# NVlabs/VILA

Measured on NVIDIA H100. Metric: NVILA-8B decode tokens/sec (1 img 448^2, bs=1, 128 new tokens); TTFT reported as ttft_ms, higher is better.
Workload: dtype bf16

## Files before the change

### vila_b200/csrc/gemm_wgmma.cu

```cuda
#include "common.cuh"
#include "kernels.h"
#include "wgmma.cuh"

namespace vb {

namespace {

constexpr int BLOCK_M = 128;
constexpr int BLOCK_K = 64;
constexpr int kConsumerThreads = 256;
constexpr int kNumThreads = kConsumerThreads + 32;

enum { kModeSingle = 0, kModePair = 1, kModeSplitK2 = 2 };

template <int BLOCK_N, int kStages, int kMode = kModeSingle>
struct GemmSmem {
  static constexpr int kABytes = BLOCK_M * BLOCK_K * 2;
  static constexpr int kBBytes = BLOCK_N * BLOCK_K * 2;
  static constexpr int kStageBytes = kABytes + kBBytes;
  static constexpr int kBarrierBytes = 2 * kStages * 8 + 16;
  static constexpr int kTotal = kStages * kStageBytes + kBarrierBytes + 1024;
  static_assert(kMode != kModeSplitK2 || BLOCK_M * BLOCK_N * 2 <= kStages * kStageBytes, "");
};

__device__ __forceinline__ float2 ld_cg_v2(const float* p) {
  float2 r;
  asm volatile("ld.global.cg.v2.f32 {%0,%1}, [%2];" : "=f"(r.x), "=f"(r.y) : "l"(p));
  return r;
}

constexpr int kBandM = 8;
__device__ __forceinline__ void tile_coords(int t, int num_m_blocks, int num_n_blocks, int& m_blk, int& n_blk) {
  const int per_band = kBandM * num_n_blocks;
  const int band = t / per_band;
  const int r = t - band * per_band;
  const int m0 = band * kBandM;
  const int bm = min(kBandM, num_m_blocks - m0);
  n_blk = r / bm;
  m_blk = m0 + (r - n_blk * bm);
}

struct Sched {
  int nkb, num_m_blocks, num_tiles;
  int stream_k;
  long it, it_end;
  int tile;
  int stride;
  __device__ __forceinline__ Sched(int M, int N, int K, int block_n, int stream_k_, int tile_m,
                                   int worker, int n_workers) {
    nkb = (K + BLOCK_K - 1) / BLOCK_K;
    num_m_blocks = (M + tile_m - 1) / tile_m;
    num_tiles = num_m_blocks * ((N + block_n - 1) / block_n);
    stream_k = stream_k_;
    const long total = static_cast<long>(num_tiles) * nkb;
    it = total * worker / n_workers;
    it_end = total * (worker + 1) / n_workers;
    tile = worker;
    stride = n_workers;
  }
  __device__ __forceinline__ bool next(int& t, int& kb0, int& kb1) {
    if (stream_k) {
      if (it >= it_end) return false;
      t = static_cast<int>(it / nkb);
      kb0 = static_cast<int>(it - static_cast<long>(t) * nkb);
      const long rem = it_end - it;
      kb1 = (nkb - kb0) < rem ? nkb : kb0 + static_cast<int>(rem);
      it += kb1 - kb0;
      return true;
    }
    if (tile >= num_tiles) return false;
    t = tile;
    kb0 = 0;
    kb1 = nkb;
    tile += stride;
    return true;
  }
};

template <int BLOCK_N>
__device__ __forceinline__ void epilogue_store(const float* acc, const GemmEpilogue& epi, __nv_bfloat16* C,
                                               int ldc, int M, int N, int row0, int n_base, int col0,
                                               int j_lo, int j_hi) {
#pragma unroll
  for (int h = 0; h < 2; ++h) {
    const int row = row0 + 8 * h;
    if (row >= M) continue;
    const __nv_bfloat16* res_row = nullptr;
    if (epi.residual != nullptr) {
      const int rr = epi.res_row_mod > 0 ? (row % epi.res_row_mod) : row;
      res_row = epi.residual + static_cast<size_t>(rr) * epi.ld_res;
    }
#pragma unroll
    for (int j = 0; j < BLOCK_N / 8; ++j) {
      if (j < j_lo || j >= j_hi) continue;
      const int n = n_base + 8 * j + col0;
      if (n >= N) continue;
      float v0 = acc[4 * j + 2 * h], v1 = acc[4 * j + 2 * h + 1];
      if (epi.bias != nullptr) {
        const uint32_t b = *reinterpret_cast<const uint32_t*>(epi.bias + n);
        v0 += bf_lo(b);
        v1 += bf_hi(b);
      }
      if (epi.swiglu) {
        const float g = bf16_round(v0), u = bf16_round(v1);
        C[static_cast<size_t>(row) * ldc + (n >> 1)] = __float2bfloat16_rn(bf16_round(silu_f(g)) * u);
        continue;
      }
      if (epi.act != ACT_NONE) {
        const float x0 = bf16_round(v0), x1 = bf16_round(v1);
        if (epi.act == ACT_GELU_TANH) {
          v0 = gelu_tanh_f(x0);
          v1 = gelu_tanh_f(x1);
        } else if (epi.act == ACT_GELU_ERF) {
          v0 = gelu_erf_f(x0);
          v1 = gelu_erf_f(x1);
        } else {
          v0 = silu_f(x0);
          v1 = silu_f(x1);
        }
      }
      if (res_row != nullptr) {
        const uint32_t r = *reinterpret_cast<const uint32_t*>(res_row + n);
        v0 = bf16_round(v0) + bf_lo(r);
        v1 = bf16_round(v1) + bf_hi(r);
      }
      *reinterpret_cast<uint32_t*>(C + static_cast<size_t>(row) * ldc + n) = pack_bf16(v0, v1);
    }
  }
}

template <int BLOCK_N, int kStages, int kMode>
__global__ void __launch_bounds__(kNumThreads, 1)
gemm_bf16_wgmma_kernel(const __grid_constant__ CUtensorMap tmap_a,
                       const __grid_constant__ CUtensorMap tmap_w, __nv_bfloat16* __restrict__ C,
                       int ldc, int M, int N, int K, GemmEpilogue epi) {
  using S = GemmSmem<BLOCK_N, kStages, kMode>;
  constexpr bool kPair = kMode == kModePair;
  constexpr bool kSplit2 = kMode == kModeSplitK2;
  constexpr bool kCluster = kPair || kSplit2;
  constexpr int TILE_M = kPair ? 2 * BLOCK_M : BLOCK_M;
  constexpr int kAcc = BLOCK_N / 2;
  extern __shared__ uint8_t smem_raw[];
  uint8_t* smem = reinterpret_cast<uint8_t*>((reinterpret_cast<uintptr_t>(smem_raw) + 1023) &
                                             ~static_cast<uintptr_t>(1023));
  uint8_t* smem_a = smem;
  uint8_t* smem_b = smem + kStages * S::kABytes;
  uint64_t* full_bar = reinterpret_cast<uint64_t*>(smem + kStages * S::kStageBytes);
  uint64_t* empty_bar = full_bar + kStages;
  uint32_t* last_flag = reinterpret_cast<uint32_t*>(empty_bar + kStages);

  const int warp = threadIdx.x >> 5;
  const int lane = threadIdx.x & 31;
  const int num_m_blocks = (M + TILE_M - 1) / TILE_M;
  const int num_n_blocks = (N + BLOCK_N - 1) / BLOCK_N;
  const int stream_k = (!kCluster && epi.split_k > 1) ? 1 : 0;
  const uint32_t rank = kCluster ? cluster_ctarank() : 0u;
  const uint32_t mrank = kPair ? rank : 0u;
  const int worker = kCluster ? static_cast<int>(blockIdx.x >> 1) : static_cast<int>(blockIdx.x);
  const int n_workers = kCluster ? static_cast<int>(gridDim.x >> 1) : static_cast<int>(gridDim.x);
  const int nkb_all = (K + BLOCK_K - 1) / BLOCK_K;
  const int sk_lo = (kSplit2 && rank == 1) ? (nkb_all + 1) / 2 : 0;
  const int sk_hi = (kSplit2 && rank == 0) ? (nkb_all + 1) / 2 : nkb_all;

  if (threadIdx.x == kConsumerThreads) {
    tma_prefetch_desc(&tmap_a);
    tma_prefetch_desc(&tmap_w);
#pragma unroll
    for (int i = 0; i < kStages; ++i) {
      mbar_init(&full_bar[i], 1);
      mbar_init(&empty_bar[i], kPair ? 4 : 2);
    }
    fence_barrier_init();
  }
  if (kCluster) cluster_sync_all();
  else __syncthreads();
  griddep_launch_dependents();

  if (warp == kConsumerThreads / 32) {
    if (lane == 0) {
      Sched sch(M, N, K, BLOCK_N, stream_k, TILE_M, worker, n_workers);
      constexpr int kWRows = kPair ? BLOCK_N / 2 : BLOCK_N;
      const int a_row_off = static_cast<int>(mrank) * BLOCK_M;
      const int w_row_off = static_cast<int>(mrank) * kWRows;
      auto load_w = [&](int stage, int kb, int n_blk) {
        uint8_t* dst = smem_b + stage * S::kBBytes + w_row_off * (BLOCK_K * 2);
        if (kPair) tma_load_2d_multicast(dst, &tmap_w, &full_bar[stage], kb * BLOCK_K, n_blk * BLOCK_N + w_row_off, 3);
        else tma_load_2d(dst, &tmap_w, &full_bar[stage], kb * BLOCK_K, n_blk * BLOCK_N);
      };
      int stage = 0;
      uint32_t phase = 0;
      int t, kb0, kb1;
      int pre = 0;
      int pt = 0, pkb0 = 0, pkb1 = 0;
      Sched peek = sch;
      const bool have_first = peek.next(pt, pkb0, pkb1);
      if (kSplit2) {
        pkb0 = sk_lo;
        pkb1 = sk_hi;
      }
      if (!kPair && epi.static_w && have_first) {
        pre = min(kStages, pkb1 - pkb0);
        int m_blk_unused, n_blk;
        tile_coords(pt, num_m_blocks, num_n_blocks, m_blk_unused, n_blk);
        for (int i = 0; i < pre; ++i) {
          mbar_arrive_expect_tx(&full_bar[i], S::kStageBytes);
          load_w(i, pkb0 + i, n_blk);
        }
      }
      griddep_wait();
      bool first = true;
      while (sch.next(t, kb0, kb1)) {
        int m_blk, n_blk;
        tile_coords(t, num_m_blocks, num_n_blocks, m_blk, n_blk);
        if (kSplit2) {
          kb0 = sk_lo;
          kb1 = sk_hi;
        }
        for (int kb = kb0; kb < kb1; ++kb) {
          if (first && (kb - kb0) < pre) {
            tma_load_2d(smem_a + stage * S::kABytes, &tmap_a, &full_bar[stage], kb * BLOCK_K,
                        m_blk * TILE_M + a_row_off);
          } else {
            mbar_wait(&empty_bar[stage], phase ^ 1);
            mbar_arrive_expect_tx(&full_bar[stage], S::kStageBytes);
            tma_load_2d(smem_a + stage * S::kABytes, &tmap_a, &full_bar[stage], kb * BLOCK_K,
                        m_blk * TILE_M + a_row_off);
            load_w(stage, kb, n_blk);
          }
          if (++stage == kStages) {
            stage = 0;
            phase ^= 1;
          }
        }
        first = false;
      }
    }
  } else {
    const int wg = warp >> 2;
    const int ctid = threadIdx.x;
    const int frag_row = wg * 64 + (warp & 3) * 16 + (lane >> 2);
    const int col0 = (lane & 3) * 2;
    Sched sch(M, N, K, BLOCK_N, stream_k, TILE_M, worker, n_workers);
    int stage = 0;
    uint32_t phase = 0;
    int t, kb0, kb1;
    float acc[kAcc];
    griddep_wait();
    while (sch.next(t, kb0, kb1)) {
      int m_blk, n_blk;
      tile_coords(t, num_m_blocks, num_n_blocks, m_blk, n_blk);
      if (kSplit2) {
        kb0 = sk_lo;
        kb1 = sk_hi;
      }
      auto release = [&](int s) {
        __syncwarp();
        if ((warp & 3) == 0 && lane == 0) {
          if (kPair) {
            mbar_arrive_cluster(mapa_u32(smem_u32(&empty_bar[s]), 0));
            mbar_arrive_cluster(mapa_u32(smem_u32(&empty_bar[s]), 1));
          } else {
            mbar_arrive(&empty_bar[s]);
          }
        }
      };
      int prev_stage = -1;
      for (int kb = kb0; kb < kb1; ++kb) {
        mbar_wait(&full_bar[stage], phase);
        wgmma_fence_operand<kAcc>(acc);
        wgmma_fence();
        const uint32_t a_base = smem_u32(smem_a + stage * S::kABytes) + wg * (64 * BLOCK_K * 2);
        const uint32_t b_base = smem_u32(smem_b + stage * S::kBBytes);
#pragma unroll
        for (int k = 0; k < BLOCK_K / 16; ++k) {
          const uint64_t ad = make_wgmma_desc(a_base + k * 32, 16, 1024, kWgmmaSW128);
          const uint64_t bd = make_wgmma_desc(b_base + k * 32, 16, 1024, kWgmmaSW128);
          Wgmma<BLOCK_N>::ss(acc, ad, bd, (kb != kb0 || k != 0) ? 1u : 0u);
        }
        wgmma_commit();
        wgmma_wait<1>();
        wgmma_fence_operand<kAcc>(acc);
        if (prev_stage >= 0) release(prev_stage);
        prev_stage = stage;
        if (++stage == kStages) {
          stage = 0;
          phase ^= 1;
        }
      }
      wgmma_wait<0>();
      wgmma_fence_operand<kAcc>(acc);
      if (prev_stage >= 0) release(prev_stage);

      const int row0 = m_blk * TILE_M + static_cast<int>(mrank) * BLOCK_M + frag_row;
      const int n_base = n_blk * BLOCK_N;
      int j_lo = 0, j_hi = BLOCK_N / 8;
      if (kSplit2) {
        named_bar_sync(1, kConsumerThreads);
        float2* xchg = reinterpret_cast<float2*>(smem_a);
        constexpr int kHalfJ = BLOCK_N / 16;
        const bool mine_low = rank == 0;
#pragma unroll
        for (int j = 0; j < BLOCK_N / 8; ++j) {
          if ((j < kHalfJ) == mine_low) continue;
#pragma unroll
          for (int h = 0; h < 2; ++h)
            xchg[((j % kHalfJ) * 2 + h) * kConsumerThreads + ctid] =
                make_float2(acc[4 * j + 2 * h], acc[4 * j + 2 * h + 1]);
        }
        cluster_sync_all();
        const uint32_t xchg_peer = mapa_u32(smem_u32(xchg), 1u - rank);
        j_lo = static_cast<int>(rank) * kHalfJ;
        j_hi = j_lo + kHalfJ;
#pragma unroll
        for (int j = 0; j < BLOCK_N / 8; ++j) {
          if ((j < kHalfJ) != mine_low) continue;
#pragma unroll
          for (int h = 0; h < 2; ++h) {
            const float2 q =
                ld_dsmem_v2f(xchg_peer + static_cast<uint32_t>(((j % kHalfJ) * 2 + h) * kConsumerThreads + ctid) * 8u);
            acc[4 * j + 2 * h] += q.x;
            acc[4 * j + 2 * h + 1] += q.y;
          }
        }
      }
      const bool partial = stream_k && ((kb0 != 0) || (kb1 != sch.nkb));
      bool finalize = true;
      if (partial) {
        const long total = static_cast<long>(sch.num_tiles) * sch.nkb;
        const long i0 = static_cast<long>(t) * sch.nkb;
        auto cta_of = [&](long i) {
          long g = i * gridDim.x / total;
          while (g + 1 < static_cast<long>(gridDim.x) && total * (g + 1) / gridDim.x <= i) ++g;
          return static_cast<int>(g);
        };
        const int c_first = cta_of(i0);
        const int n_slots = cta_of(i0 + sch.nkb - 1) - c_first + 1;
        const int my_slot = static_cast<int>(blockIdx.x) - c_first;
        const size_t tile_base = static_cast<size_t>(t) * epi.split_k * (BLOCK_M * BLOCK_N);
        float* slot0 = epi.splitk_ws + tile_base;
        float* mine = slot0 + static_cast<size_t>(my_slot) * (BLOCK_M * BLOCK_N);
#pragma unroll
        for (int j = 0; j < BLOCK_N / 8; ++j)
#pragma unroll
          for (int h = 0; h < 2; ++h)
            if (row0 + 8 * h < M)
              *reinterpret_cast<float2*>(mine + (frag_row + 8 * h) * BLOCK_N + 8 * j + col0) =
                  make_float2(acc[4 * j + 2 * h], acc[4 * j + 2 * h + 1]);
        __threadfence();
        named_bar_sync(1, kConsumerThreads);
        if (ctid == 0) {
          const int add = kb1 - kb0;
          const int prev = atomicAdd(&epi.splitk_counters[t], add);
          const int last = (prev + add == sch.nkb) ? 1 : 0;
          if (last) epi.splitk_counters[t] = 0;
          *last_flag = last;
        }
        named_bar_sync(1, kConsumerThreads);
        finalize = (*last_flag != 0);
        named_bar_sync(1, kConsumerThreads);
        if (finalize) {
          __threadfence();
#pragma unroll
          for (int i = 0; i < kAcc; ++i) acc[i] = 0.f;
          for (int s = 0; s < n_slots; ++s) {
            const float* wsp = slot0 + static_cast<size_t>(s) * (BLOCK_M * BLOCK_N);
#pragma unroll
            for (int j = 0; j < BLOCK_N / 8; ++j)
#pragma unroll
              for (int h = 0; h < 2; ++h) {
                if (row0 + 8 * h >= M) continue;
                const float2 q = ld_cg_v2(wsp + (frag_row + 8 * h) * BLOCK_N + 8 * j + col0);
                acc[4 * j + 2 * h] += q.x;
                acc[4 * j + 2 * h + 1] += q.y;
              }
          }
        }
      }
      if (finalize) epilogue_store<BLOCK_N>(acc, epi, C, ldc, M, N, row0, n_base, col0, j_lo, j_hi);
    }
  }

  if (kSplit2 && warp == kConsumerThreads / 32) cluster_sync_all();
  if (kCluster) cluster_sync_all();
}

struct Workspace {
  void* ptr = nullptr;
  size_t bytes = 0;
};
Workspace g_ws_dev[64];
inline Workspace& cur_ws() {
  int d = 0;
  cudaGetDevice(&d);
  return g_ws_dev[(d < 0 || d >= 64) ? 0 : d];
}
#define g_ws cur_ws()
constexpr size_t kCounterBytes = 64 * 1024;

template <int BLOCK_N, int kStages, int kMode = kModeSingle>
int launch_gemm(const __nv_bfloat16* A, int lda, const __nv_bfloat16* W, int ldw, __nv_bfloat16* C,
                int ldc, int M, int N, int K, GemmEpilogue epi, int force_stream_k,
                cudaStream_t stream) {
  using S = GemmSmem<BLOCK_N, kStages, kMode>;
  constexpr bool kPair = kMode == kModePair;
  constexpr int TILE_M = kPair ? 2 * BLOCK_M : BLOCK_M;
  CUtensorMap ta, tw;
  if (make_tmap_2d_bf16(&ta, A, M, K, lda, BLOCK_M, BLOCK_K, 128)) return 1;
  if (make_tmap_2d_bf16(&tw, W, N, K, ldw, kPair ? BLOCK_N / 2 : BLOCK_N, BLOCK_K, 128)) return 1;
  auto kern = gemm_bf16_wgmma_kernel<BLOCK_N, kStages, kMode>;
  static PerDeviceOnce attr_once;
  if (attr_once.first()) {
    VB_CUDA(cudaFuncSetAttribute(kern, cudaFuncAttributeMaxDynamicSharedMemorySize, S::kTotal));
  }
  const int sms = num_sms();
  const int tiles = ((M + TILE_M - 1) / TILE_M) * ((N + BLOCK_N - 1) / BLOCK_N);
  if (kMode == kModeSplitK2) {
    if ((K + BLOCK_K - 1) / BLOCK_K < 2) {
      set_last_error("gemm: split-K pairs need >= 2 k-blocks (K=%d)", K);
      return 1;
    }
    epi.split_k = 1;
    VB_CUDA(launch_pdl_cluster(kern, dim3(2 * tiles), dim3(kNumThreads), S::kTotal, stream,
                               dim3(2, 1, 1), ta, tw, C, ldc, M, N, K, epi));
    return 0;
  }
  if (kPair) {
    const int pairs = tiles < sms / 2 ? tiles : sms / 2;
    epi.split_k = 1;
    VB_CUDA(launch_pdl_cluster(kern, dim3(2 * pairs), dim3(kNumThreads), S::kTotal, stream,
                               dim3(2, 1, 1), ta, tw, C, ldc, M, N, K, epi));
    return 0;
  }
  const int nkb = (K + BLOCK_K - 1) / BLOCK_K;
  bool sk = false;
  const long total_it = static_cast<long>(tiles) * nkb;
  const int sk_grid = total_it < sms ? static_cast<int>(total_it) : sms;
  const long ipc = total_it / sk_grid;
  const int max_slots = static_cast<int>((nkb + ipc - 1) / ipc) + 1;
  const size_t need = kCounterBytes + static_cast<size_t>(tiles) * max_slots * BLOCK_M * BLOCK_N * 4;
  const bool ws_ok = g_ws.ptr != nullptr && g_ws.bytes >= need && tiles <= 16384;
  if (force_stream_k == 2) {
    sk = ws_ok;
  } else if (force_stream_k >= 0) {
    sk = force_stream_k != 0;
  }
  if (sk && !ws_ok) {
    set_last_error("gemm: stream-K needs a registered workspace of >= %zu bytes (vila_set_workspace)",
                   need);
    return 1;
  }
  int grid = tiles < sms ? tiles : sms;
  epi.split_k = 1;
  if (sk) {
    grid = sk_grid;
    epi.split_k = max_slots;
    epi.splitk_counters = static_cast<int*>(g_ws.ptr);
    epi.splitk_ws = reinterpret_cast<float*>(static_cast<char*>(g_ws.ptr) + kCounterBytes);
  }
  VB_CUDA(launch_pdl(kern, dim3(grid), dim3(kNumThreads), S::kTotal, stream, ta, tw, C, ldc, M, N,
                     K, epi));
  return 0;
}

int check_args(const __nv_bfloat16* A, int lda, const __nv_bfloat16* W, int ldw, __nv_bfloat16* C,
               int ldc, int M, int N, int K, const GemmEpilogue& epi) {
  VB_CHECK(M > 0 && N > 0 && K > 0, "gemm: empty problem M=%d N=%d K=%d", M, N, K);
  VB_CHECK(K % 8 == 0 && lda % 8 == 0 && ldw % 8 == 0,
           "gemm: K, lda, ldw must be multiples of 8 (TMA 16-byte strides): K=%d lda=%d ldw=%d", K,
           lda, ldw);
  VB_CHECK(N % 8 == 0 && ldc % 8 == 0, "gemm: N and ldc must be multiples of 8: N=%d ldc=%d", N,
           ldc);
  VB_CHECK((reinterpret_cast<uintptr_t>(A) & 15) == 0 && (reinterpret_cast<uintptr_t>(W) & 15) == 0 &&
               (reinterpret_cast<uintptr_t>(C) & 15) == 0,
           "gemm: pointers must be 16-byte aligned");
  if (epi.swiglu) VB_CHECK(N % 32 == 0, "gemm: swiglu epilogue needs N %% 32 == 0 (N=%d)", N);
  return 0;
}

int gemm_skinny(const __nv_bfloat16* A, int lda, const __nv_bfloat16* W, int ldw, __nv_bfloat16* C,
                int ldc, int M, int N, int K, const GemmEpilogue& epi, int pair, cudaStream_t stream) {
  if (pair) return launch_gemm<128, 6, kModePair>(A, lda, W, ldw, C, ldc, M, N, K, epi, -1, stream);
  return launch_gemm<128, 6>(A, lda, W, ldw, C, ldc, M, N, K, epi, -1, stream);
}

}

int gemm_qkv_rope_bf16(const __nv_bfloat16* A, int lda, const __nv_bfloat16* W, int ldw, __nv_bfloat16* C,
                       int ldc, int M, int N, int K, const GemmEpilogue& epi, cudaStream_t stream) {
  if (check_args(A, lda, W, ldw, C, ldc, M, N, K, epi)) return 1;
  if (M > 384) return -1;
  VB_CHECK(ldc == N, "gemm_qkv_rope: the q/k/v output must be dense (ldc %d != N %d)", ldc, N);
  GemmEpilogue plain;
  plain.bias = epi.bias;
  plain.static_w = epi.static_w;
  const int rc = gemm_skinny(A, lda, W, ldw, C, ldc, M, N, K, plain, 0, stream);
  if (rc != 0) return rc;
  return rope_kv_append_table(C, epi.rope_table, M, epi.rope_hq, epi.rope_hkv, 128, epi.k_pool, epi.v_pool,
                              epi.page_table, epi.cache_pos0, stream);
}

void get_workspace(void** ptr, size_t* bytes) {
  *ptr = g_ws.ptr;
  *bytes = g_ws.bytes;
}

int set_workspace(void* ptr, size_t bytes) {
  VB_CHECK(ptr == nullptr || bytes >= kCounterBytes + 1024, "workspace too small (%zu bytes)", bytes);
  VB_CHECK((reinterpret_cast<uintptr_t>(ptr) & 255) == 0, "workspace must be 256-byte aligned");
  g_ws.ptr = ptr;
  g_ws.bytes = ptr ? bytes : 0;
  return 0;
}

int gemm_bf16(const __nv_bfloat16* A, int lda, const __nv_bfloat16* W, int ldw, __nv_bfloat16* C,
              int ldc, int M, int N, int K, const GemmEpilogue& epi, cudaStream_t stream) {
  if (check_args(A, lda, W, ldw, C, ldc, M, N, K, epi)) return 1;
  VB_CHECK(epi.rope_table == nullptr, "gemm: the fused RoPE epilogue is only available through gemm_qkv_rope_bf16");
  const int sms = num_sms();
  const int mb = (M + BLOCK_M - 1) / BLOCK_M;
  const long tiles128 = static_cast<long>(mb) * ((N + 127) / 128);
  const bool split2 = tiles128 <= sms / 2 && K >= 2048 && M * 10 >= mb * BLOCK_M * 9;
  if (split2) return launch_gemm<128, 6, kModeSplitK2>(A, lda, W, ldw, C, ldc, M, N, K, epi, -1, stream);
  if (K >= 8192 && tiles128 < sms) {
    if (tiles128 * 2 <= sms) return launch_gemm<128, 6>(A, lda, W, ldw, C, ldc, M, N, K, epi, 2, stream);
    return launch_gemm<128, 6, kModeSplitK2>(A, lda, W, ldw, C, ldc, M, N, K, epi, -1, stream);
  }
  const long tiles256 = static_cast<long>(mb) * ((N + 255) / 256);
  if (tiles256 * 10 >= 7L * sms)
    return launch_gemm<256, 4>(A, lda, W, ldw, C, ldc, M, N, K, epi, -1, stream);
  if (N < 128) return launch_gemm<64, 8>(A, lda, W, ldw, C, ldc, M, N, K, epi, -1, stream);
  return launch_gemm<128, 6>(A, lda, W, ldw, C, ldc, M, N, K, epi, -1, stream);
}

int gemm_bf16_cfg(int block_n, const __nv_bfloat16* A, int lda, const __nv_bfloat16* W, int ldw,
                  __nv_bfloat16* C, int ldc, int M, int N, int K, const GemmEpilogue& epi,
                  cudaStream_t stream) {
  if (check_args(A, lda, W, ldw, C, ldc, M, N, K, epi)) return 1;
  if (block_n == 4256) return launch_gemm<256, 4, kModePair>(A, lda, W, ldw, C, ldc, M, N, K, epi, -1, stream);
  if (block_n == 4128) return launch_gemm<128, 6, kModePair>(A, lda, W, ldw, C, ldc, M, N, K, epi, -1, stream);
  if (block_n == 5128) return launch_gemm<128, 6, kModeSplitK2>(A, lda, W, ldw, C, ldc, M, N, K, epi, -1, stream);
  if (block_n == 3000 || block_n == 3001) {
    VB_CHECK(M <= 512, "gemm_bf16_cfg: the skinny path handles M <= 512 (M=%d)", M);
    return gemm_skinny(A, lda, W, ldw, C, ldc, M, N, K, epi, block_n - 3000, stream);
  }
  int fsk = -1;
  if (block_n >= 2000) {
    fsk = 0;
    block_n -= 2000;
  } else if (block_n >= 1000) {
    fsk = 1;
    block_n -= 1000;
  }
  switch (block_n) {
    case 64: return launch_gemm<64, 8>(A, lda, W, ldw, C, ldc, M, N, K, epi, fsk, stream);
    case 128: return launch_gemm<128, 6>(A, lda, W, ldw, C, ldc, M, N, K, epi, fsk, stream);
    case 256: return launch_gemm<256, 4>(A, lda, W, ldw, C, ldc, M, N, K, epi, fsk, stream);
    default: set_last_error("gemm_bf16_cfg: unsupported block_n %d", block_n); return 1;
  }
}

}
```

### vila_b200/csrc/wgmma.cuh

```cuda
#pragma once
#include <stdint.h>

namespace vb {

__device__ __forceinline__ void wgmma_fence() { asm volatile("wgmma.fence.sync.aligned;" ::: "memory"); }
__device__ __forceinline__ void wgmma_commit() { asm volatile("wgmma.commit_group.sync.aligned;" ::: "memory"); }
template <int kPending>
__device__ __forceinline__ void wgmma_wait() {
  asm volatile("wgmma.wait_group.sync.aligned %0;" ::"n"(kPending) : "memory");
}
template <int kN>
__device__ __forceinline__ void wgmma_fence_operand(float* d) {
#pragma unroll
  for (int i = 0; i < kN; ++i) asm volatile("" : "+f"(d[i])::"memory");
}

template <int N> struct Wgmma;

template <>
struct Wgmma<64> {
  __device__ __forceinline__ static void ss(float* d, uint64_t a, uint64_t b, uint32_t acc) {
    asm volatile(
        "{\n.reg .pred p;\nsetp.ne.b32 p, %34, 0;\n"
        "wgmma.mma_async.sync.aligned.m64n64k16.f32.bf16.bf16 {%0,%1,%2,%3,%4,%5,%6,%7,%8,%9,%10,%11,%12,%13,%14,%15,%16,%17,%18,%19,%20,%21,%22,%23,%24,%25,%26,%27,%28,%29,%30,%31}, %32, %33, p, 1, 1, 0, 0;\n}\n"
        : "+f"(d[0]), "+f"(d[1]), "+f"(d[2]), "+f"(d[3]), "+f"(d[4]), "+f"(d[5]), "+f"(d[6]), "+f"(d[7]), "+f"(d[8]), "+f"(d[9]), "+f"(d[10]), "+f"(d[11]), "+f"(d[12]), "+f"(d[13]), "+f"(d[14]), "+f"(d[15]), "+f"(d[16]), "+f"(d[17]), "+f"(d[18]), "+f"(d[19]), "+f"(d[20]), "+f"(d[21]), "+f"(d[22]), "+f"(d[23]), "+f"(d[24]), "+f"(d[25]), "+f"(d[26]), "+f"(d[27]), "+f"(d[28]), "+f"(d[29]), "+f"(d[30]), "+f"(d[31])
        : "l"(a), "l"(b), "r"(acc));
  }
  __device__ __forceinline__ static void rs_bt(float* d, const uint32_t* a, uint64_t b) {
    asm volatile(
        "{\n.reg .pred p;\nsetp.ne.b32 p, %37, 0;\n"
        "wgmma.mma_async.sync.aligned.m64n64k16.f32.bf16.bf16 {%0,%1,%2,%3,%4,%5,%6,%7,%8,%9,%10,%11,%12,%13,%14,%15,%16,%17,%18,%19,%20,%21,%22,%23,%24,%25,%26,%27,%28,%29,%30,%31}, {%32,%33,%34,%35}, %36, p, 1, 1, 1;\n}\n"
        : "+f"(d[0]), "+f"(d[1]), "+f"(d[2]), "+f"(d[3]), "+f"(d[4]), "+f"(d[5]), "+f"(d[6]), "+f"(d[7]), "+f"(d[8]), "+f"(d[9]), "+f"(d[10]), "+f"(d[11]), "+f"(d[12]), "+f"(d[13]), "+f"(d[14]), "+f"(d[15]), "+f"(d[16]), "+f"(d[17]), "+f"(d[18]), "+f"(d[19]), "+f"(d[20]), "+f"(d[21]), "+f"(d[22]), "+f"(d[23]), "+f"(d[24]), "+f"(d[25]), "+f"(d[26]), "+f"(d[27]), "+f"(d[28]), "+f"(d[29]), "+f"(d[30]), "+f"(d[31])
        : "r"(a[0]), "r"(a[1]), "r"(a[2]), "r"(a[3]), "l"(b), "n"(1));
  }
};

template <>
struct Wgmma<96> {
  __device__ __forceinline__ static void ss(float* d, uint64_t a, uint64_t b, uint32_t acc) {
    asm volatile(
        "{\n.reg .pred p;\nsetp.ne.b32 p, %50, 0;\n"
        "wgmma.mma_async.sync.aligned.m64n96k16.f32.bf16.bf16 {%0,%1,%2,%3,%4,%5,%6,%7,%8,%9,%10,%11,%12,%13,%14,%15,%16,%17,%18,%19,%20,%21,%22,%23,%24,%25,%26,%27,%28,%29,%30,%31,%32,%33,%34,%35,%36,%37,%38,%39,%40,%41,%42,%43,%44,%45,%46,%47}, %48, %49, p, 1, 1, 0, 0;\n}\n"
        : "+f"(d[0]), "+f"(d[1]), "+f"(d[2]), "+f"(d[3]), "+f"(d[4]), "+f"(d[5]), "+f"(d[6]), "+f"(d[7]), "+f"(d[8]), "+f"(d[9]), "+f"(d[10]), "+f"(d[11]), "+f"(d[12]), "+f"(d[13]), "+f"(d[14]), "+f"(d[15]), "+f"(d[16]), "+f"(d[17]), "+f"(d[18]), "+f"(d[19]), "+f"(d[20]), "+f"(d[21]), "+f"(d[22]), "+f"(d[23]), "+f"(d[24]), "+f"(d[25]), "+f"(d[26]), "+f"(d[27]), "+f"(d[28]), "+f"(d[29]), "+f"(d[30]), "+f"(d[31]), "+f"(d[32]), "+f"(d[33]), "+f"(d[34]), "+f"(d[35]), "+f"(d[36]), "+f"(d[37]), "+f"(d[38]), "+f"(d[39]), "+f"(d[40]), "+f"(d[41]), "+f"(d[42]), "+f"(d[43]), "+f"(d[44]), "+f"(d[45]), "+f"(d[46]), "+f"(d[47])
        : "l"(a), "l"(b), "r"(acc));
  }
  __device__ __forceinline__ static void rs_bt(float* d, const uint32_t* a, uint64_t b) {
    asm volatile(
        "{\n.reg .pred p;\nsetp.ne.b32 p, %53, 0;\n"
        "wgmma.mma_async.sync.aligned.m64n96k16.f32.bf16.bf16 {%0,%1,%2,%3,%4,%5,%6,%7,%8,%9,%10,%11,%12,%13,%14,%15,%16,%17,%18,%19,%20,%21,%22,%23,%24,%25,%26,%27,%28,%29,%30,%31,%32,%33,%34,%35,%36,%37,%38,%39,%40,%41,%42,%43,%44,%45,%46,%47}, {%48,%49,%50,%51}, %52, p, 1, 1, 1;\n}\n"
        : "+f"(d[0]), "+f"(d[1]), "+f"(d[2]), "+f"(d[3]), "+f"(d[4]), "+f"(d[5]), "+f"(d[6]), "+f"(d[7]), "+f"(d[8]), "+f"(d[9]), "+f"(d[10]), "+f"(d[11]), "+f"(d[12]), "+f"(d[13]), "+f"(d[14]), "+f"(d[15]), "+f"(d[16]), "+f"(d[17]), "+f"(d[18]), "+f"(d[19]), "+f"(d[20]), "+f"(d[21]), "+f"(d[22]), "+f"(d[23]), "+f"(d[24]), "+f"(d[25]), "+f"(d[26]), "+f"(d[27]), "+f"(d[28]), "+f"(d[29]), "+f"(d[30]), "+f"(d[31]), "+f"(d[32]), "+f"(d[33]), "+f"(d[34]), "+f"(d[35]), "+f"(d[36]), "+f"(d[37]), "+f"(d[38]), "+f"(d[39]), "+f"(d[40]), "+f"(d[41]), "+f"(d[42]), "+f"(d[43]), "+f"(d[44]), "+f"(d[45]), "+f"(d[46]), "+f"(d[47])
        : "r"(a[0]), "r"(a[1]), "r"(a[2]), "r"(a[3]), "l"(b), "n"(1));
  }
};

template <>
struct Wgmma<128> {
  __device__ __forceinline__ static void ss(float* d, uint64_t a, uint64_t b, uint32_t acc) {
    asm volatile(
        "{\n.reg .pred p;\nsetp.ne.b32 p, %66, 0;\n"
        "wgmma.mma_async.sync.aligned.m64n128k16.f32.bf16.bf16 {%0,%1,%2,%3,%4,%5,%6,%7,%8,%9,%10,%11,%12,%13,%14,%15,%16,%17,%18,%19,%20,%21,%22,%23,%24,%25,%26,%27,%28,%29,%30,%31,%32,%33,%34,%35,%36,%37,%38,%39,%40,%41,%42,%43,%44,%45,%46,%47,%48,%49,%50,%51,%52,%53,%54,%55,%56,%57,%58,%59,%60,%61,%62,%63}, %64, %65, p, 1, 1, 0, 0;\n}\n"
        : "+f"(d[0]), "+f"(d[1]), "+f"(d[2]), "+f"(d[3]), "+f"(d[4]), "+f"(d[5]), "+f"(d[6]), "+f"(d[7]), "+f"(d[8]), "+f"(d[9]), "+f"(d[10]), "+f"(d[11]), "+f"(d[12]), "+f"(d[13]), "+f"(d[14]), "+f"(d[15]), "+f"(d[16]), "+f"(d[17]), "+f"(d[18]), "+f"(d[19]), "+f"(d[20]), "+f"(d[21]), "+f"(d[22]), "+f"(d[23]), "+f"(d[24]), "+f"(d[25]), "+f"(d[26]), "+f"(d[27]), "+f"(d[28]), "+f"(d[29]), "+f"(d[30]), "+f"(d[31]), "+f"(d[32]), "+f"(d[33]), "+f"(d[34]), "+f"(d[35]), "+f"(d[36]), "+f"(d[37]), "+f"(d[38]), "+f"(d[39]), "+f"(d[40]), "+f"(d[41]), "+f"(d[42]), "+f"(d[43]), "+f"(d[44]), "+f"(d[45]), "+f"(d[46]), "+f"(d[47]), "+f"(d[48]), "+f"(d[49]), "+f"(d[50]), "+f"(d[51]), "+f"(d[52]), "+f"(d[53]), "+f"(d[54]), "+f"(d[55]), "+f"(d[56]), "+f"(d[57]), "+f"(d[58]), "+f"(d[59]), "+f"(d[60]), "+f"(d[61]), "+f"(d[62]), "+f"(d[63])
        : "l"(a), "l"(b), "r"(acc));
  }
  __device__ __forceinline__ static void rs_bt(float* d, const uint32_t* a, uint64_t b) {
    asm volatile(
        "{\n.reg .pred p;\nsetp.ne.b32 p, %69, 0;\n"
        "wgmma.mma_async.sync.aligned.m64n128k16.f32.bf16.bf16 {%0,%1,%2,%3,%4,%5,%6,%7,%8,%9,%10,%11,%12,%13,%14,%15,%16,%17,%18,%19,%20,%21,%22,%23,%24,%25,%26,%27,%28,%29,%30,%31,%32,%33,%34,%35,%36,%37,%38,%39,%40,%41,%42,%43,%44,%45,%46,%47,%48,%49,%50,%51,%52,%53,%54,%55,%56,%57,%58,%59,%60,%61,%62,%63}, {%64,%65,%66,%67}, %68, p, 1, 1, 1;\n}\n"
        : "+f"(d[0]), "+f"(d[1]), "+f"(d[2]), "+f"(d[3]), "+f"(d[4]), "+f"(d[5]), "+f"(d[6]), "+f"(d[7]), "+f"(d[8]), "+f"(d[9]), "+f"(d[10]), "+f"(d[11]), "+f"(d[12]), "+f"(d[13]), "+f"(d[14]), "+f"(d[15]), "+f"(d[16]), "+f"(d[17]), "+f"(d[18]), "+f"(d[19]), "+f"(d[20]), "+f"(d[21]), "+f"(d[22]), "+f"(d[23]), "+f"(d[24]), "+f"(d[25]), "+f"(d[26]), "+f"(d[27]), "+f"(d[28]), "+f"(d[29]), "+f"(d[30]), "+f"(d[31]), "+f"(d[32]), "+f"(d[33]), "+f"(d[34]), "+f"(d[35]), "+f"(d[36]), "+f"(d[37]), "+f"(d[38]), "+f"(d[39]), "+f"(d[40]), "+f"(d[41]), "+f"(d[42]), "+f"(d[43]), "+f"(d[44]), "+f"(d[45]), "+f"(d[46]), "+f"(d[47]), "+f"(d[48]), "+f"(d[49]), "+f"(d[50]), "+f"(d[51]), "+f"(d[52]), "+f"(d[53]), "+f"(d[54]), "+f"(d[55]), "+f"(d[56]), "+f"(d[57]), "+f"(d[58]), "+f"(d[59]), "+f"(d[60]), "+f"(d[61]), "+f"(d[62]), "+f"(d[63])
        : "r"(a[0]), "r"(a[1]), "r"(a[2]), "r"(a[3]), "l"(b), "n"(1));
  }
};

template <>
struct Wgmma<256> {
  __device__ __forceinline__ static void ss(float* d, uint64_t a, uint64_t b, uint32_t acc) {
    asm volatile(
        "{\n.reg .pred p;\nsetp.ne.b32 p, %130, 0;\n"
        "wgmma.mma_async.sync.aligned.m64n256k16.f32.bf16.bf16 {%0,%1,%2,%3,%4,%5,%6,%7,%8,%9,%10,%11,%12,%13,%14,%15,%16,%17,%18,%19,%20,%21,%22,%23,%24,%25,%26,%27,%28,%29,%30,%31,%32,%33,%34,%35,%36,%37,%38,%39,%40,%41,%42,%43,%44,%45,%46,%47,%48,%49,%50,%51,%52,%53,%54,%55,%56,%57,%58,%59,%60,%61,%62,%63,%64,%65,%66,%67,%68,%69,%70,%71,%72,%73,%74,%75,%76,%77,%78,%79,%80,%81,%82,%83,%84,%85,%86,%87,%88,%89,%90,%91,%92,%93,%94,%95,%96,%97,%98,%99,%100,%101,%102,%103,%104,%105,%106,%107,%108,%109,%110,%111,%112,%113,%114,%115,%116,%117,%118,%119,%120,%121,%122,%123,%124,%125,%126,%127}, %128, %129, p, 1, 1, 0, 0;\n}\n"
        : "+f"(d[0]), "+f"(d[1]), "+f"(d[2]), "+f"(d[3]), "+f"(d[4]), "+f"(d[5]), "+f"(d[6]), "+f"(d[7]), "+f"(d[8]), "+f"(d[9]), "+f"(d[10]), "+f"(d[11]), "+f"(d[12]), "+f"(d[13]), "+f"(d[14]), "+f"(d[15]), "+f"(d[16]), "+f"(d[17]), "+f"(d[18]), "+f"(d[19]), "+f"(d[20]), "+f"(d[21]), "+f"(d[22]), "+f"(d[23]), "+f"(d[24]), "+f"(d[25]), "+f"(d[26]), "+f"(d[27]), "+f"(d[28]), "+f"(d[29]), "+f"(d[30]), "+f"(d[31]), "+f"(d[32]), "+f"(d[33]), "+f"(d[34]), "+f"(d[35]), "+f"(d[36]), "+f"(d[37]), "+f"(d[38]), "+f"(d[39]), "+f"(d[40]), "+f"(d[41]), "+f"(d[42]), "+f"(d[43]), "+f"(d[44]), "+f"(d[45]), "+f"(d[46]), "+f"(d[47]), "+f"(d[48]), "+f"(d[49]), "+f"(d[50]), "+f"(d[51]), "+f"(d[52]), "+f"(d[53]), "+f"(d[54]), "+f"(d[55]), "+f"(d[56]), "+f"(d[57]), "+f"(d[58]), "+f"(d[59]), "+f"(d[60]), "+f"(d[61]), "+f"(d[62]), "+f"(d[63]), "+f"(d[64]), "+f"(d[65]), "+f"(d[66]), "+f"(d[67]), "+f"(d[68]), "+f"(d[69]), "+f"(d[70]), "+f"(d[71]), "+f"(d[72]), "+f"(d[73]), "+f"(d[74]), "+f"(d[75]), "+f"(d[76]), "+f"(d[77]), "+f"(d[78]), "+f"(d[79]), "+f"(d[80]), "+f"(d[81]), "+f"(d[82]), "+f"(d[83]), "+f"(d[84]), "+f"(d[85]), "+f"(d[86]), "+f"(d[87]), "+f"(d[88]), "+f"(d[89]), "+f"(d[90]), "+f"(d[91]), "+f"(d[92]), "+f"(d[93]), "+f"(d[94]), "+f"(d[95]), "+f"(d[96]), "+f"(d[97]), "+f"(d[98]), "+f"(d[99]), "+f"(d[100]), "+f"(d[101]), "+f"(d[102]), "+f"(d[103]), "+f"(d[104]), "+f"(d[105]), "+f"(d[106]), "+f"(d[107]), "+f"(d[108]), "+f"(d[109]), "+f"(d[110]), "+f"(d[111]), "+f"(d[112]), "+f"(d[113]), "+f"(d[114]), "+f"(d[115]), "+f"(d[116]), "+f"(d[117]), "+f"(d[118]), "+f"(d[119]), "+f"(d[120]), "+f"(d[121]), "+f"(d[122]), "+f"(d[123]), "+f"(d[124]), "+f"(d[125]), "+f"(d[126]), "+f"(d[127])
        : "l"(a), "l"(b), "r"(acc));
  }
  __device__ __forceinline__ static void rs_bt(float* d, const uint32_t* a, uint64_t b) {
    asm volatile(
        "{\n.reg .pred p;\nsetp.ne.b32 p, %133, 0;\n"
        "wgmma.mma_async.sync.aligned.m64n256k16.f32.bf16.bf16 {%0,%1,%2,%3,%4,%5,%6,%7,%8,%9,%10,%11,%12,%13,%14,%15,%16,%17,%18,%19,%20,%21,%22,%23,%24,%25,%26,%27,%28,%29,%30,%31,%32,%33,%34,%35,%36,%37,%38,%39,%40,%41,%42,%43,%44,%45,%46,%47,%48,%49,%50,%51,%52,%53,%54,%55,%56,%57,%58,%59,%60,%61,%62,%63,%64,%65,%66,%67,%68,%69,%70,%71,%72,%73,%74,%75,%76,%77,%78,%79,%80,%81,%82,%83,%84,%85,%86,%87,%88,%89,%90,%91,%92,%93,%94,%95,%96,%97,%98,%99,%100,%101,%102,%103,%104,%105,%106,%107,%108,%109,%110,%111,%112,%113,%114,%115,%116,%117,%118,%119,%120,%121,%122,%123,%124,%125,%126,%127}, {%128,%129,%130,%131}, %132, p, 1, 1, 1;\n}\n"
        : "+f"(d[0]), "+f"(d[1]), "+f"(d[2]), "+f"(d[3]), "+f"(d[4]), "+f"(d[5]), "+f"(d[6]), "+f"(d[7]), "+f"(d[8]), "+f"(d[9]), "+f"(d[10]), "+f"(d[11]), "+f"(d[12]), "+f"(d[13]), "+f"(d[14]), "+f"(d[15]), "+f"(d[16]), "+f"(d[17]), "+f"(d[18]), "+f"(d[19]), "+f"(d[20]), "+f"(d[21]), "+f"(d[22]), "+f"(d[23]), "+f"(d[24]), "+f"(d[25]), "+f"(d[26]), "+f"(d[27]), "+f"(d[28]), "+f"(d[29]), "+f"(d[30]), "+f"(d[31]), "+f"(d[32]), "+f"(d[33]), "+f"(d[34]), "+f"(d[35]), "+f"(d[36]), "+f"(d[37]), "+f"(d[38]), "+f"(d[39]), "+f"(d[40]), "+f"(d[41]), "+f"(d[42]), "+f"(d[43]), "+f"(d[44]), "+f"(d[45]), "+f"(d[46]), "+f"(d[47]), "+f"(d[48]), "+f"(d[49]), "+f"(d[50]), "+f"(d[51]), "+f"(d[52]), "+f"(d[53]), "+f"(d[54]), "+f"(d[55]), "+f"(d[56]), "+f"(d[57]), "+f"(d[58]), "+f"(d[59]), "+f"(d[60]), "+f"(d[61]), "+f"(d[62]), "+f"(d[63]), "+f"(d[64]), "+f"(d[65]), "+f"(d[66]), "+f"(d[67]), "+f"(d[68]), "+f"(d[69]), "+f"(d[70]), "+f"(d[71]), "+f"(d[72]), "+f"(d[73]), "+f"(d[74]), "+f"(d[75]), "+f"(d[76]), "+f"(d[77]), "+f"(d[78]), "+f"(d[79]), "+f"(d[80]), "+f"(d[81]), "+f"(d[82]), "+f"(d[83]), "+f"(d[84]), "+f"(d[85]), "+f"(d[86]), "+f"(d[87]), "+f"(d[88]), "+f"(d[89]), "+f"(d[90]), "+f"(d[91]), "+f"(d[92]), "+f"(d[93]), "+f"(d[94]), "+f"(d[95]), "+f"(d[96]), "+f"(d[97]), "+f"(d[98]), "+f"(d[99]), "+f"(d[100]), "+f"(d[101]), "+f"(d[102]), "+f"(d[103]), "+f"(d[104]), "+f"(d[105]), "+f"(d[106]), "+f"(d[107]), "+f"(d[108]), "+f"(d[109]), "+f"(d[110]), "+f"(d[111]), "+f"(d[112]), "+f"(d[113]), "+f"(d[114]), "+f"(d[115]), "+f"(d[116]), "+f"(d[117]), "+f"(d[118]), "+f"(d[119]), "+f"(d[120]), "+f"(d[121]), "+f"(d[122]), "+f"(d[123]), "+f"(d[124]), "+f"(d[125]), "+f"(d[126]), "+f"(d[127])
        : "r"(a[0]), "r"(a[1]), "r"(a[2]), "r"(a[3]), "l"(b), "n"(1));
  }
};

}
```

Before: 182.6.

## Add swap-AB skinny GEMM path with narrow token tiles and split-K modes

Adds a swap-AB variant of the WGMMA GEMM for small M: weights take the 128-row MMA M slot and tokens take the N slot, using new n32/n144 wgmma shapes. The epilogue uses a lane shuffle to re-pair the transposed accumulators. A heuristic picks whole-tile, stream-K or split-K pair scheduling, and the main gemm entry now routes small-M calls to this path. The goal is to avoid wasting most of a 128-row M tile on decode-sized token counts, at the cost of more template instantiations and new epilogue indexing that could be wrong.

After: 182.5, median of 6. About the same (-0.0%).

```diff
diff --git a/vila_b200/csrc/gemm_wgmma.cu b/vila_b200/csrc/gemm_wgmma.cu
--- a/vila_b200/csrc/gemm_wgmma.cu
+++ b/vila_b200/csrc/gemm_wgmma.cu
@@ -1,3 +1,5 @@
+#include <utility>
+
 #include "common.cuh"
 #include "kernels.h"
 #include "wgmma.cuh"
@@ -77,6 +79,46 @@
   }
 };
 
+__device__ __forceinline__ const __nv_bfloat16* residual_row(const GemmEpilogue& epi, int row) {
+  if (epi.residual == nullptr) return nullptr;
+  const int rr = epi.res_row_mod > 0 ? (row % epi.res_row_mod) : row;
+  return epi.residual + static_cast<size_t>(rr) * epi.ld_res;
+}
+
+__device__ __forceinline__ void epilogue_pair(const GemmEpilogue& epi, __nv_bfloat16* C, int ldc,
+                                              const __nv_bfloat16* res_row, int row, int n, float v0,
+                                              float v1) {
+  if (epi.bias != nullptr) {
+    const uint32_t b = *reinterpret_cast<const uint32_t*>(epi.bias + n);
+    v0 += bf_lo(b);
+    v1 += bf_hi(b);
+  }
+  if (epi.swiglu) {
+    const float g = bf16_round(v0), u = bf16_round(v1);
+    C[static_cast<size_t>(row) * ldc + (n >> 1)] = __float2bfloat16_rn(bf16_round(silu_f(g)) * u);
+    return;
+  }
+  if (epi.act != ACT_NONE) {
+    const float x0 = bf16_round(v0), x1 = bf16_round(v1);
+    if (epi.act == ACT_GELU_TANH) {
+      v0 = gelu_tanh_f(x0);
+      v1 = gelu_tanh_f(x1);
+    } else if (epi.act == ACT_GELU_ERF) {
+      v0 = gelu_erf_f(x0);
+      v1 = gelu_erf_f(x1);
+    } else {
+      v0 = silu_f(x0);
+      v1 = silu_f(x1);
+    }
+  }
+  if (res_row != nullptr) {
+    const uint32_t r = *reinterpret_cast<const uint32_t*>(res_row + n);
+    v0 = bf16_round(v0) + bf_lo(r);
+    v1 = bf16_round(v1) + bf_hi(r);
+  }
+  *reinterpret_cast<uint32_t*>(C + static_cast<size_t>(row) * ldc + n) = pack_bf16(v0, v1);
+}
+
 template <int BLOCK_N>
 __device__ __forceinline__ void epilogue_store(const float* acc, const GemmEpilogue& epi, __nv_bfloat16* C,
                                                int ldc, int M, int N, int row0, int n_base, int col0,
@@ -85,51 +127,39 @@
   for (int h = 0; h < 2; ++h) {
     const int row = row0 + 8 * h;
     if (row >= M) continue;
-    const __nv_bfloat16* res_row = nullptr;
-    if (epi.residual != nullptr) {
-      const int rr = epi.res_row_mod > 0 ? (row % epi.res_row_mod) : row;
-      res_row = epi.residual + static_cast<size_t>(rr) * epi.ld_res;
-    }
+    const __nv_bfloat16* res_row = residual_row(epi, row);
 #pragma unroll
     for (int j = 0; j < BLOCK_N / 8; ++j) {
       if (j < j_lo || j >= j_hi) continue;
       const int n = n_base + 8 * j + col0;
       if (n >= N) continue;
-      float v0 = acc[4 * j + 2 * h], v1 = acc[4 * j + 2 * h + 1];
-      if (epi.bias != nullptr) {
-        const uint32_t b = *reinterpret_cast<const uint32_t*>(epi.bias + n);
-        v0 += bf_lo(b);
-        v1 += bf_hi(b);
-      }
-      if (epi.swiglu) {
-        const float g = bf16_round(v0), u = bf16_round(v1);
-        C[static_cast<size_t>(row) * ldc + (n >> 1)] = __float2bfloat16_rn(bf16_round(silu_f(g)) * u);
-        continue;
-      }
-      if (epi.act != ACT_NONE) {
-        const float x0 = bf16_round(v0), x1 = bf16_round(v1);
-        if (epi.act == ACT_GELU_TANH) {
-          v0 = gelu_tanh_f(x0);
-          v1 = gelu_tanh_f(x1);
-        } else if (epi.act == ACT_GELU_ERF) {
-          v0 = gelu_erf_f(x0);
-          v1 = gelu_erf_f(x1);
-        } else {
-          v0 = silu_f(x0);
-          v1 = silu_f(x1);
-        }
-      }
-      if (res_row != nullptr) {
-        const uint32_t r = *reinterpret_cast<const uint32_t*>(res_row + n);
-        v0 = bf16_round(v0) + bf_lo(r);
-        v1 = bf16_round(v1) + bf_hi(r);
-      }
-      *reinterpret_cast<uint32_t*>(C + static_cast<size_t>(row) * ldc + n) = pack_bf16(v0, v1);
-    }
-  }
-}
-
-template <int BLOCK_N, int kStages, int kMode>
+      epilogue_pair(epi, C, ldc, res_row, row, n, acc[4 * j + 2 * h], acc[4 * j + 2 * h + 1]);
+    }
+  }
+}
+
+template <int TN>
+__device__ __forceinline__ void epilogue_store_swap(const float* acc, const GemmEpilogue& epi, __nv_bfloat16* C,
+                                                    int ldc, int n_out, int m_tok, int n_row0, int tok_base,
+                                                    int col0, int lane, int j_lo, int j_hi) {
+  const int odd = (lane >> 2) & 1;
+#pragma unroll
+  for (int h = 0; h < 2; ++h) {
+    const int n = n_row0 + 8 * h - odd;
+#pragma unroll
+    for (int j = 0; j < TN / 8; ++j) {
+      if (j < j_lo || j >= j_hi) continue;
+      const float a0 = acc[4 * j + 2 * h], a1 = acc[4 * j + 2 * h + 1];
+      const float other = __shfl_xor_sync(0xffffffffu, odd ? a0 : a1, 4);
+      const int tok = tok_base + 8 * j + col0 + odd;
+      if (tok >= m_tok || n >= n_out) continue;
+      const float v0 = odd ? other : a0, v1 = odd ? a1 : other;
+      epilogue_pair(epi, C, ldc, residual_row(epi, tok), tok, n, v0, v1);
+    }
+  }
+}
+
+template <int BLOCK_N, int kStages, int kMode, bool kSwap>
 __global__ void __launch_bounds__(kNumThreads, 1)
 gemm_bf16_wgmma_kernel(const __grid_constant__ CUtensorMap tmap_a,
                        const __grid_constant__ CUtensorMap tmap_w, __nv_bfloat16* __restrict__ C,
@@ -182,6 +212,10 @@
       constexpr int kWRows = kPair ? BLOCK_N / 2 : BLOCK_N;
       const int a_row_off = static_cast<int>(mrank) * BLOCK_M;
       const int w_row_off = static_cast<int>(mrank) * kWRows;
+      auto load_a = [&](int stage, int kb, int m_blk) {
+        tma_load_2d(smem_a + stage * S::kABytes, &tmap_a, &full_bar[stage], kb * BLOCK_K,
+                    m_blk * TILE_M + a_row_off);
+      };
       auto load_w = [&](int stage, int kb, int n_blk) {
         uint8_t* dst = smem_b + stage * S::kBBytes + w_row_off * (BLOCK_K * 2);
         if (kPair) tma_load_2d_multicast(dst, &tmap_w, &full_bar[stage], kb * BLOCK_K, n_blk * BLOCK_N + w_row_off, 3);
@@ -200,11 +234,12 @@
       }
       if (!kPair && epi.static_w && have_first) {
         pre = min(kStages, pkb1 - pkb0);
-        int m_blk_unused, n_blk;
-        tile_coords(pt, num_m_blocks, num_n_blocks, m_blk_unused, n_blk);
+        int m_blk, n_blk;
+        tile_coords(pt, num_m_blocks, num_n_blocks, m_blk, n_blk);
         for (int i = 0; i < pre; ++i) {
           mbar_arrive_expect_tx(&full_bar[i], S::kStageBytes);
-          load_w(i, pkb0 + i, n_blk);
+          if (kSwap) load_a(i, pkb0 + i, m_blk);
+          else load_w(i, pkb0 + i, n_blk);
         }
       }
       griddep_wait();
@@ -218,13 +253,12 @@
         }
         for (int kb = kb0; kb < kb1; ++kb) {
           if (first && (kb - kb0) < pre) {
-            tma_load_2d(smem_a + stage * S::kABytes, &tmap_a, &full_bar[stage], kb * BLOCK_K,
-                        m_blk * TILE_M + a_row_off);
+            if (kSwap) load_w(stage, kb, n_blk);
+            else load_a(stage, kb, m_blk);
           } else {
             mbar_wait(&empty_bar[stage], phase ^ 1);
             mbar_arrive_expect_tx(&full_bar[stage], S::kStageBytes);
-            tma_load_2d(smem_a + stage * S::kABytes, &tmap_a, &full_bar[stage], kb * BLOCK_K,
-                        m_blk * TILE_M + a_row_off);
+            load_a(stage, kb, m_blk);
             load_w(stage, kb, n_blk);
           }
           if (++stage == kStages) {
@@ -376,7 +410,10 @@
           }
         }
       }
-      if (finalize) epilogue_store<BLOCK_N>(acc, epi, C, ldc, M, N, row0, n_base, col0, j_lo, j_hi);
+      if (finalize) {
+        if (kSwap) epilogue_store_swap<BLOCK_N>(acc, epi, C, ldc, M, N, row0, n_base, col0, lane, j_lo, j_hi);
+        else epilogue_store<BLOCK_N>(acc, epi, C, ldc, M, N, row0, n_base, col0, j_lo, j_hi);
+      }
     }
   }
 
@@ -397,17 +434,22 @@
 #define g_ws cur_ws()
 constexpr size_t kCounterBytes = 64 * 1024;
 
-template <int BLOCK_N, int kStages, int kMode = kModeSingle>
+template <int BLOCK_N, int kStages, int kMode = kModeSingle, bool kSwap = false>
 int launch_gemm(const __nv_bfloat16* A, int lda, const __nv_bfloat16* W, int ldw, __nv_bfloat16* C,
                 int ldc, int M, int N, int K, GemmEpilogue epi, int force_stream_k,
                 cudaStream_t stream) {
   using S = GemmSmem<BLOCK_N, kStages, kMode>;
   constexpr bool kPair = kMode == kModePair;
   constexpr int TILE_M = kPair ? 2 * BLOCK_M : BLOCK_M;
+  if (kSwap) {
+    std::swap(A, W);
+    std::swap(lda, ldw);
+    std::swap(M, N);
+  }
   CUtensorMap ta, tw;
   if (make_tmap_2d_bf16(&ta, A, M, K, lda, BLOCK_M, BLOCK_K, 128)) return 1;
   if (make_tmap_2d_bf16(&tw, W, N, K, ldw, kPair ? BLOCK_N / 2 : BLOCK_N, BLOCK_K, 128)) return 1;
-  auto kern = gemm_bf16_wgmma_kernel<BLOCK_N, kStages, kMode>;
+  auto kern = gemm_bf16_wgmma_kernel<BLOCK_N, kStages, kMode, kSwap>;
   static PerDeviceOnce attr_once;
   if (attr_once.first()) {
     VB_CUDA(cudaFuncSetAttribute(kern, cudaFuncAttributeMaxDynamicSharedMemorySize, S::kTotal));
@@ -477,10 +519,39 @@
   return 0;
 }
 
+enum SkinnyMode { kSkWhole = 0, kSkStreamK = 1, kSkSplitPairs = 2, kSkCtaPairs = 3 };
+
+template <int TN, int kStages>
+int launch_swap(const __nv_bfloat16* A, int lda, const __nv_bfloat16* W, int ldw, __nv_bfloat16* C,
+                int ldc, int M, int N, int K, const GemmEpilogue& epi, int mode, cudaStream_t stream) {
+  if (mode == kSkCtaPairs)
+    return launch_gemm<TN, kStages, kModePair, true>(A, lda, W, ldw, C, ldc, M, N, K, epi, -1, stream);
+  if (mode == kSkSplitPairs)
+    return launch_gemm<TN, kStages, kModeSplitK2, true>(A, lda, W, ldw, C, ldc, M, N, K, epi, -1, stream);
+  return launch_gemm<TN, kStages, kModeSingle, true>(A, lda, W, ldw, C, ldc, M, N, K, epi,
+                                                     mode == kSkStreamK ? 2 : -1, stream);
+}
+
+int skinny_tn(int M) {
+  if (M <= 64) return M <= 32 ? 32 : 64;
+  return (M + 143) / 144 * 144 < (M + 127) / 128 * 128 ? 144 : 128;
+}
+
 int gemm_skinny(const __nv_bfloat16* A, int lda, const __nv_bfloat16* W, int ldw, __nv_bfloat16* C,
-                int ldc, int M, int N, int K, const GemmEpilogue& epi, int pair, cudaStream_t stream) {
-  if (pair) return launch_gemm<128, 6, kModePair>(A, lda, W, ldw, C, ldc, M, N, K, epi, -1, stream);
-  return launch_gemm<128, 6>(A, lda, W, ldw, C, ldc, M, N, K, epi, -1, stream);
+                int ldc, int M, int N, int K, const GemmEpilogue& epi, int mode, cudaStream_t stream) {
+  switch (skinny_tn(M)) {
+    case 32: return launch_swap<32, 8>(A, lda, W, ldw, C, ldc, M, N, K, epi, mode, stream);
+    case 64: return launch_swap<64, 8>(A, lda, W, ldw, C, ldc, M, N, K, epi, mode, stream);
+    case 128: return launch_swap<128, 6>(A, lda, W, ldw, C, ldc, M, N, K, epi, mode, stream);
+    default: return launch_swap<144, 6>(A, lda, W, ldw, C, ldc, M, N, K, epi, mode, stream);
+  }
+}
+
+int skinny_mode(int M, int N, int K) {
+  const long tiles128 = static_cast<long>((M + BLOCK_M - 1) / BLOCK_M) * ((N + 127) / 128);
+  const int sms = num_sms();
+  if (K < 8192 || tiles128 >= sms) return kSkWhole;
+  return tiles128 * 2 <= sms ? kSkStreamK : kSkSplitPairs;
 }
 
 }
@@ -493,7 +564,7 @@
   GemmEpilogue plain;
   plain.bias = epi.bias;
   plain.static_w = epi.static_w;
-  const int rc = gemm_skinny(A, lda, W, ldw, C, ldc, M, N, K, plain, 0, stream);
+  const int rc = gemm_skinny(A, lda, W, ldw, C, ldc, M, N, K, plain, skinny_mode(M, N, K), stream);
   if (rc != 0) return rc;
   return rope_kv_append_table(C, epi.rope_table, M, epi.rope_hq, epi.rope_hkv, 128, epi.k_pool, epi.v_pool,
                               epi.page_table, epi.cache_pos0, stream);
@@ -517,6 +588,8 @@
   if (check_args(A, lda, W, ldw, C, ldc, M, N, K, epi)) return 1;
   VB_CHECK(epi.rope_table == nullptr, "gemm: the fused RoPE epilogue is only available through gemm_qkv_rope_bf16");
   const int sms = num_sms();
+  if (M <= 384 && (M <= 64 || M > 256 || N >= BLOCK_M * sms))
+    return gemm_skinny(A, lda, W, ldw, C, ldc, M, N, K, epi, skinny_mode(M, N, K), stream);
   const int mb = (M + BLOCK_M - 1) / BLOCK_M;
   const long tiles128 = static_cast<long>(mb) * ((N + 127) / 128);
   const bool split2 = tiles128 <= sms / 2 && K >= 2048 && M * 10 >= mb * BLOCK_M * 9;
@@ -539,9 +612,11 @@
   if (block_n == 4256) return launch_gemm<256, 4, kModePair>(A, lda, W, ldw, C, ldc, M, N, K, epi, -1, stream);
   if (block_n == 4128) return launch_gemm<128, 6, kModePair>(A, lda, W, ldw, C, ldc, M, N, K, epi, -1, stream);
   if (block_n == 5128) return launch_gemm<128, 6, kModeSplitK2>(A, lda, W, ldw, C, ldc, M, N, K, epi, -1, stream);
-  if (block_n == 3000 || block_n == 3001) {
-    VB_CHECK(M <= 512, "gemm_bf16_cfg: the skinny path handles M <= 512 (M=%d)", M);
-    return gemm_skinny(A, lda, W, ldw, C, ldc, M, N, K, epi, block_n - 3000, stream);
+  if (block_n >= 3000 && block_n <= 3004) {
+    VB_CHECK(M <= 512, "gemm_bf16_cfg: the swap-AB path handles M <= 512 (M=%d)", M);
+    static const int kHookMode[] = {-1, kSkCtaPairs, kSkWhole, kSkStreamK, kSkSplitPairs};
+    const int mode = block_n == 3000 ? skinny_mode(M, N, K) : kHookMode[block_n - 3000];
+    return gemm_skinny(A, lda, W, ldw, C, ldc, M, N, K, epi, mode, stream);
   }
   int fsk = -1;
   if (block_n >= 2000) {
diff --git a/vila_b200/csrc/wgmma.cuh b/vila_b200/csrc/wgmma.cuh
--- a/vila_b200/csrc/wgmma.cuh
+++ b/vila_b200/csrc/wgmma.cuh
@@ -16,6 +16,17 @@
 }
 
 template <int N> struct Wgmma;
+
+template <>
+struct Wgmma<32> {
+  __device__ __forceinline__ static void ss(float* d, uint64_t a, uint64_t b, uint32_t acc) {
+    asm volatile(
+        "{\n.reg .pred p;\nsetp.ne.b32 p, %18, 0;\n"
+        "wgmma.mma_async.sync.aligned.m64n32k16.f32.bf16.bf16 {%0,%1,%2,%3,%4,%5,%6,%7,%8,%9,%10,%11,%12,%13,%14,%15}, %16, %17, p, 1, 1, 0, 0;\n}\n"
+        : "+f"(d[0]), "+f"(d[1]), "+f"(d[2]), "+f"(d[3]), "+f"(d[4]), "+f"(d[5]), "+f"(d[6]), "+f"(d[7]), "+f"(d[8]), "+f"(d[9]), "+f"(d[10]), "+f"(d[11]), "+f"(d[12]), "+f"(d[13]), "+f"(d[14]), "+f"(d[15])
+        : "l"(a), "l"(b), "r"(acc));
+  }
+};
 
 template <>
 struct Wgmma<64> {
@@ -72,6 +83,17 @@
 };
 
 template <>
+struct Wgmma<144> {
+  __device__ __forceinline__ static void ss(float* d, uint64_t a, uint64_t b, uint32_t acc) {
+    asm volatile(
+        "{\n.reg .pred p;\nsetp.ne.b32 p, %74, 0;\n"
+        "wgmma.mma_async.sync.aligned.m64n144k16.f32.bf16.bf16 {%0,%1,%2,%3,%4,%5,%6,%7,%8,%9,%10,%11,%12,%13,%14,%15,%16,%17,%18,%19,%20,%21,%22,%23,%24,%25,%26,%27,%28,%29,%30,%31,%32,%33,%34,%35,%36,%37,%38,%39,%40,%41,%42,%43,%44,%45,%46,%47,%48,%49,%50,%51,%52,%53,%54,%55,%56,%57,%58,%59,%60,%61,%62,%63,%64,%65,%66,%67,%68,%69,%70,%71}, %72, %73, p, 1, 1, 0, 0;\n}\n"
+        : "+f"(d[0]), "+f"(d[1]), "+f"(d[2]), "+f"(d[3]), "+f"(d[4]), "+f"(d[5]), "+f"(d[6]), "+f"(d[7]), "+f"(d[8]), "+f"(d[9]), "+f"(d[10]), "+f"(d[11]), "+f"(d[12]), "+f"(d[13]), "+f"(d[14]), "+f"(d[15]), "+f"(d[16]), "+f"(d[17]), "+f"(d[18]), "+f"(d[19]), "+f"(d[20]), "+f"(d[21]), "+f"(d[22]), "+f"(d[23]), "+f"(d[24]), "+f"(d[25]), "+f"(d[26]), "+f"(d[27]), "+f"(d[28]), "+f"(d[29]), "+f"(d[30]), "+f"(d[31]), "+f"(d[32]), "+f"(d[33]), "+f"(d[34]), "+f"(d[35]), "+f"(d[36]), "+f"(d[37]), "+f"(d[38]), "+f"(d[39]), "+f"(d[40]), "+f"(d[41]), "+f"(d[42]), "+f"(d[43]), "+f"(d[44]), "+f"(d[45]), "+f"(d[46]), "+f"(d[47]), "+f"(d[48]), "+f"(d[49]), "+f"(d[50]), "+f"(d[51]), "+f"(d[52]), "+f"(d[53]), "+f"(d[54]), "+f"(d[55]), "+f"(d[56]), "+f"(d[57]), "+f"(d[58]), "+f"(d[59]), "+f"(d[60]), "+f"(d[61]), "+f"(d[62]), "+f"(d[63]), "+f"(d[64]), "+f"(d[65]), "+f"(d[66]), "+f"(d[67]), "+f"(d[68]), "+f"(d[69]), "+f"(d[70]), "+f"(d[71])
+        : "l"(a), "l"(b), "r"(acc));
+  }
+};
+
+template <>
 struct Wgmma<256> {
   __device__ __forceinline__ static void ss(float* d, uint64_t a, uint64_t b, uint32_t acc) {
     asm volatile(
```
